# dfki-asr/morphablegraphs

Measured on AMD Instinct MI355X. Metric: motion-primitive samples scored+back-projected/sec; fraction of HBM roofline, higher is better.
Workload: dtype f32; 1 GPU; walk primitive L=40 F=156 D=79 NB=31 GMM k=8, batch=8192 candidates/GPU (BASELINE.json configs[1]); candidates_per_gpu=8192, global_candidates=8192, collective=none, clock_ramp_steps=1500

## Files before the change

morphablegraphs_amd/csrc/mg_frames_direct.hip:

```cpp
#include "mg_frames_common.h"

struct mg_direct_args {
    const float *Et32;
    const double *Et64;
    const double *mean;
    const void *lat;
    const int32_t *i0;
    const double *w;
    const float *rootm;
    void *out;
    int64_t B, ld;
    int32_t T, D, L, R, nroot;
    int32_t split;
};

template <bool LAT_F64, bool OUT_F64>
__global__ __launch_bounds__(256) void mg_frames_direct_kernel(mg_direct_args a) {
    const int64_t TD = (int64_t)a.T * a.D;
    const int64_t total = a.B * TD;
    for (int64_t idx = (int64_t)blockIdx.x * blockDim.x + threadIdx.x; idx < total; idx += (int64_t)gridDim.x * blockDim.x) {
        const int64_t b = idx / TD;
        const int o = (int)(idx - b * TD);
        const int f = o / a.D, d = o - f * a.D;
        const int i0v = a.i0[f];
        const double *wq = a.w + 4 * (size_t)f;
        const int r0 = i0v * a.D + d;
        if (!OUT_F64 && d < a.nroot && a.split) {
            float c[4];
#pragma unroll
            for (int j = 0; j < 4; j++) {
                const float *e = a.Et32 + (r0 + j * a.D);
                float acc = 0.0f;
                for (int k = 0; k < a.L; k++) acc = fmaf(e[(size_t)k * a.R], (float)mg_load_lat<LAT_F64>(a.lat, b * a.ld + k), acc);
                c[j] = acc;
            }
            float v = (float)wq[0] * c[0];
            v = fmaf((float)wq[1], c[1], v);
            v = fmaf((float)wq[2], c[2], v);
            v = fmaf((float)wq[3], c[3], v);
            const float *m = a.rootm + 8 * (size_t)f;
            ((float *)a.out)[idx] = m[d] + (m[3 + d] + v);
        } else if (OUT_F64 || d < a.nroot) {
            double c[4];
#pragma unroll
            for (int j = 0; j < 4; j++) {
                const double *e = a.Et64 + (r0 + j * a.D);
                double acc = a.mean[r0 + j * a.D];
                for (int k = 0; k < a.L; k++) acc = fma(e[(size_t)k * a.R], mg_load_lat<LAT_F64>(a.lat, b * a.ld + k), acc);
                c[j] = acc;
            }
            double v = wq[0] * c[0];
            v = fma(wq[1], c[1], v);
            v = fma(wq[2], c[2], v);
            v = fma(wq[3], c[3], v);
            if (OUT_F64) ((double *)a.out)[idx] = v;
            else ((float *)a.out)[idx] = (float)v;
        } else {
            float c[4];
#pragma unroll
            for (int j = 0; j < 4; j++) {
                const float *e = a.Et32 + (r0 + j * a.D);
                float acc = (float)a.mean[r0 + j * a.D];
                for (int k = 0; k < a.L; k++) acc = fmaf(e[(size_t)k * a.R], (float)mg_load_lat<LAT_F64>(a.lat, b * a.ld + k), acc);
                c[j] = acc;
            }
            float v = (float)wq[0] * c[0];
            v = fmaf((float)wq[1], c[1], v);
            v = fmaf((float)wq[2], c[2], v);
            v = fmaf((float)wq[3], c[3], v);
            ((float *)a.out)[idx] = v;
        }
    }
}

__global__ __launch_bounds__(256) void mg_spline_eval_kernel(const double *coeffs, const int32_t *i0, const double *w,
                                                             double *out, int64_t n, int32_t T, int32_t D, int32_t R) {
    const int64_t TD = (int64_t)T * D, total = n * TD;
    for (int64_t idx = (int64_t)blockIdx.x * blockDim.x + threadIdx.x; idx < total; idx += (int64_t)gridDim.x * blockDim.x) {
        const int64_t s = idx / TD;
        const int o = (int)(idx - s * TD);
        const int f = o / D, d = o - f * D;
        const double *c = coeffs + s * R + (size_t)i0[f] * D + d;
        const double *wq = w + 4 * (size_t)f;
        double v = wq[0] * c[0];
        v = fma(wq[1], c[D], v);
        v = fma(wq[2], c[2 * D], v);
        v = fma(wq[3], c[3 * D], v);
        out[idx] = v;
    }
}


int mg_launch_frames_direct(mg_primitive *p, const mg_time_grid *g, const void *lat, int ldt, int64_t B, int64_t ld, void *out, bool out_f64) {
    mg_direct_args a;
    a.Et32 = p->d_Et32; a.Et64 = p->d_Et64; a.mean = p->d_mean; a.lat = lat; a.i0 = g->d_i0; a.w = g->d_w; a.out = out;
    a.rootm = g->d_rootm; a.split = (!out_f64 && mg_frames_root_split(p)) ? 1 : 0;
    a.B = B; a.ld = ld; a.T = g->T; a.D = p->D; a.L = p->L; a.R = p->R; a.nroot = p->nroot;
    int64_t total = B * (int64_t)g->T * p->D;
    int64_t blocks = (total + 255) / 256;
    int grid = (int)std::min<int64_t>(blocks, (int64_t)p->ctx->n_cu * 32);
    hipStream_t st = p->ctx->stream;
    const bool lf = (ldt == MG_F64);
    if (lf && out_f64) hipLaunchKernelGGL((mg_frames_direct_kernel<true, true>), dim3(grid), dim3(256), 0, st, a);
    else if (lf) hipLaunchKernelGGL((mg_frames_direct_kernel<true, false>), dim3(grid), dim3(256), 0, st, a);
    else if (out_f64) hipLaunchKernelGGL((mg_frames_direct_kernel<false, true>), dim3(grid), dim3(256), 0, st, a);
    else hipLaunchKernelGGL((mg_frames_direct_kernel<false, false>), dim3(grid), dim3(256), 0, st, a);
    MG_HIP_CHECK(hipGetLastError());
    return MG_OK;
}

int mg_launch_spline_eval(mg_primitive *p, const mg_time_grid *g, const double *coeffs, int64_t n, double *out) {
    int64_t total = n * (int64_t)g->T * p->D;
    int grid = (int)std::min<int64_t>((total + 255) / 256, (int64_t)p->ctx->n_cu * 32);
    hipLaunchKernelGGL(mg_spline_eval_kernel, dim3(grid), dim3(256), 0, p->ctx->stream, coeffs, g->d_i0, g->d_w, out, n, g->T, p->D, p->R);
    MG_HIP_CHECK(hipGetLastError());
    return MG_OK;
}
```

Before: 108.5 million samples/s.

## Add LDS-staged batched f64 frame kernel that reuses coefficients across candidates

Adds a new f64-output path in which each block handles up to four candidates. The block stages their latents and the spline weights in LDS, computes the full coefficient vector (mean plus Et·z) once per candidate into LDS, then evaluates the 4-tap spline from LDS with paired 16-byte stores. Before, every output element recomputed four L-length dot products from global memory. This removes that redundant FMA and load traffic, at the cost of large LDS use (up to 80KB), lower occupancy and a one-time attribute setup. It only runs when the output is f64 and the batch is at least 64.

```diff
diff --git a/morphablegraphs_amd/csrc/mg_frames_direct.hip b/morphablegraphs_amd/csrc/mg_frames_direct.hip
--- a/morphablegraphs_amd/csrc/mg_frames_direct.hip
+++ b/morphablegraphs_amd/csrc/mg_frames_direct.hip
@@ -71,6 +71,166 @@
             ((float *)a.out)[idx] = v;
         }
     }
+}
+
+#define MG_F64B_BLOCK 512
+#define MG_F64B_MAX_C 4
+#define MG_F64B_RJ 2
+#define MG_F64B_KU 8
+#define MG_F64B_MIN_BATCH 64
+#define MG_F64B_LDS_BUDGET (80 * 1024)
+
+typedef double f64x2 __attribute__((ext_vector_type(2)));
+
+static size_t mg_f64b_lds_bytes(int C, int T, int L, int R) {
+    const int CP = (C + 1) & ~1;
+    return (size_t)T * 32 + (size_t)L * CP * 8 + (size_t)C * R * 8 + (size_t)T * 4;
+}
+
+__device__ __forceinline__ double mg_f64b_tap(const double *cb, const double *ws, const int *off, int f, int d, int D) {
+    const f64x2 w01 = *(const f64x2 *)(ws + 4 * f), w23 = *(const f64x2 *)(ws + 4 * f + 2);
+    const double *c = cb + off[f] + d;
+    double v = w01[0] * c[0];
+    v = fma(w01[1], c[D], v);
+    v = fma(w23[0], c[2 * D], v);
+    v = fma(w23[1], c[3 * D], v);
+    return v;
+}
+
+template <int C, bool LAT_F64>
+__global__ __launch_bounds__(MG_F64B_BLOCK) void mg_frames_f64_batch_kernel(const double *__restrict__ Et64,
+                                                                            const double *__restrict__ mean,
+                                                                            const void *__restrict__ lat, const int32_t *__restrict__ i0,
+                                                                            const double *__restrict__ w, double *__restrict__ out,
+                                                                            int64_t B, int64_t ld, int T, int D, int L, int R) {
+    constexpr int CP = (C + 1) & ~1;
+    extern __shared__ __attribute__((aligned(16))) unsigned char smem[];
+    double *ws = (double *)smem;
+    double *s = ws + 4 * (size_t)T;
+    double *cp = s + (size_t)L * CP;
+    int *off = (int *)(cp + (size_t)C * R);
+    const int tid = threadIdx.x;
+    const int64_t b0 = (int64_t)blockIdx.x * C;
+    const int nc = (int)((B - b0) < C ? (B - b0) : C);
+    for (int i = tid; i < L * CP; i += MG_F64B_BLOCK) {
+        const int k = i / CP, c = i - k * CP;
+        s[i] = c < nc ? mg_load_lat<LAT_F64>(lat, (b0 + c) * ld + k) : 0.0;
+    }
+    for (int f = tid; f < T; f += MG_F64B_BLOCK) {
+        off[f] = i0[f] * D;
+#pragma unroll
+        for (int q = 0; q < 4; q++) ws[4 * f + q] = w[4 * (size_t)f + q];
+    }
+    __syncthreads();
+    for (int rb = 0; rb < R; rb += MG_F64B_BLOCK * MG_F64B_RJ) {
+        int r[MG_F64B_RJ];
+        double acc[MG_F64B_RJ][C];
+#pragma unroll
+        for (int j = 0; j < MG_F64B_RJ; j++) {
+            const int rj = rb + j * MG_F64B_BLOCK + tid;
+            r[j] = rj < R ? rj : R - 1;
+            const double m = mean[r[j]];
+#pragma unroll
+            for (int c = 0; c < C; c++) acc[j][c] = m;
+        }
+        auto steps = [&](const double *e, int k, auto ku) {
+            constexpr int KU = decltype(ku)::value;
+            double ev[KU][MG_F64B_RJ];
+#pragma unroll
+            for (int u = 0; u < KU; u++)
+#pragma unroll
+                for (int j = 0; j < MG_F64B_RJ; j++) ev[u][j] = e[(size_t)u * R + r[j]];
+#pragma unroll
+            for (int u = 0; u < KU; u++) {
+                f64x2 sv[CP / 2];
+#pragma unroll
+                for (int q = 0; q < CP / 2; q++) sv[q] = *(const f64x2 *)(s + (k + u) * CP + 2 * q);
+#pragma unroll
+                for (int j = 0; j < MG_F64B_RJ; j++)
+#pragma unroll
+                    for (int c = 0; c < C; c++) acc[j][c] = fma(ev[u][j], sv[c >> 1][c & 1], acc[j][c]);
+            }
+        };
+        const double *e = Et64;
+        int k = 0;
+        for (; k + MG_F64B_KU <= L; k += MG_F64B_KU, e += (size_t)MG_F64B_KU * R) steps(e, k, std::integral_constant<int, MG_F64B_KU>());
+        for (; k < L; k++, e += R) steps(e, k, std::integral_constant<int, 1>());
+#pragma unroll
+        for (int j = 0; j < MG_F64B_RJ; j++) {
+            if (rb + j * MG_F64B_BLOCK + tid < R) {
+#pragma unroll
+                for (int c = 0; c < C; c++) cp[(size_t)c * R + r[j]] = acc[j][c];
+            }
+        }
+    }
+    __syncthreads();
+    const int TD = T * D;
+    const int sf = (2 * MG_F64B_BLOCK) / D, sd = 2 * MG_F64B_BLOCK - sf * D;
+    for (int c = 0; c < nc; c++) {
+        double *ob = out + (b0 + c) * (int64_t)TD;
+        const double *cb = cp + (size_t)c * R;
+        const int head = (int)(((uintptr_t)ob >> 3) & 1);
+        const int npairs = (TD - head) >> 1;
+        if (tid == MG_F64B_BLOCK - 1 && head) ob[0] = mg_f64b_tap(cb, ws, off, 0, 0, D);
+        if (tid == MG_F64B_BLOCK - 2 && ((TD - head) & 1)) ob[TD - 1] = mg_f64b_tap(cb, ws, off, T - 1, D - 1, D);
+        int e = head + 2 * tid;
+        int f = e / D, d = e - f * D;
+        for (int p = tid; p < npairs; p += MG_F64B_BLOCK) {
+            int f1 = f, d1 = d + 1;
+            if (d1 == D) { d1 = 0; f1++; }
+            f64x2 v;
+            v[0] = mg_f64b_tap(cb, ws, off, f, d, D);
+            v[1] = mg_f64b_tap(cb, ws, off, f1, d1, D);
+            *(f64x2 *)(ob + e) = v;
+            e += 2 * MG_F64B_BLOCK;
+            f += sf; d += sd;
+            if (d >= D) { d -= D; f++; }
+        }
+    }
+}
+
+static int mg_f64b_candidates(const mg_primitive *p, const mg_time_grid *g, int64_t B) {
+    if (B < MG_F64B_MIN_BATCH || (int64_t)g->T * p->D > (int64_t)INT32_MAX / 2) return 0;
+    int cmax = 0;
+    for (int c = 1; c <= MG_F64B_MAX_C; c++)
+        if (mg_f64b_lds_bytes(c, g->T, p->L, p->R) <= MG_F64B_LDS_BUDGET) cmax = c;
+    if (cmax == 0) return 0;
+    const int64_t per_cu = B / std::max(1, p->ctx->n_cu);
+    return (int)std::min<int64_t>(cmax, std::max<int64_t>(1, per_cu));
+}
+
+template <int C>
+static void mg_f64b_launch(mg_primitive *p, const mg_time_grid *g, const void *lat, bool lat_f64, int64_t B, int64_t ld, double *out) {
+    const size_t lds = mg_f64b_lds_bytes(C, g->T, p->L, p->R);
+    const unsigned grid = (unsigned)((B + C - 1) / C);
+#define MG_F64B_ARGS (const double *)p->d_Et64, (const double *)p->d_mean, lat, (const int32_t *)g->d_i0, (const double *)g->d_w, out, B, ld, (int)g->T, (int)p->D, (int)p->L, (int)p->R
+    if (lat_f64) hipLaunchKernelGGL((mg_frames_f64_batch_kernel<C, true>), dim3(grid), dim3(MG_F64B_BLOCK), lds, p->ctx->stream, MG_F64B_ARGS);
+    else hipLaunchKernelGGL((mg_frames_f64_batch_kernel<C, false>), dim3(grid), dim3(MG_F64B_BLOCK), lds, p->ctx->stream, MG_F64B_ARGS);
+#undef MG_F64B_ARGS
+}
+
+template <int C>
+static hipError_t mg_f64b_attributes() {
+    hipError_t e = hipFuncSetAttribute((const void *)mg_frames_f64_batch_kernel<C, true>, hipFuncAttributeMaxDynamicSharedMemorySize, MG_F64B_LDS_BUDGET);
+    if (e != hipSuccess) return e;
+    return hipFuncSetAttribute((const void *)mg_frames_f64_batch_kernel<C, false>, hipFuncAttributeMaxDynamicSharedMemorySize, MG_F64B_LDS_BUDGET);
+}
+
+static int mg_launch_frames_f64_batch(mg_primitive *p, const mg_time_grid *g, const void *lat, int ldt, int64_t B, int64_t ld, double *out, int C) {
+    if (!(p->ctx->attr_traj & 16u)) {
+        MG_HIP_CHECK(mg_f64b_attributes<1>());
+        MG_HIP_CHECK(mg_f64b_attributes<2>());
+        MG_HIP_CHECK(mg_f64b_attributes<3>());
+        MG_HIP_CHECK(mg_f64b_attributes<4>());
+        p->ctx->attr_traj |= 16u;
+    }
+    const bool lf = (ldt == MG_F64);
+    if (C == 1) mg_f64b_launch<1>(p, g, lat, lf, B, ld, out);
+    else if (C == 2) mg_f64b_launch<2>(p, g, lat, lf, B, ld, out);
+    else if (C == 3) mg_f64b_launch<3>(p, g, lat, lf, B, ld, out);
+    else mg_f64b_launch<4>(p, g, lat, lf, B, ld, out);
+    MG_HIP_CHECK(hipGetLastError());
+    return MG_OK;
 }
 
 __global__ __launch_bounds__(256) void mg_spline_eval_kernel(const double *coeffs, const int32_t *i0, const double *w,
@@ -92,6 +252,10 @@
 
 
 int mg_launch_frames_direct(mg_primitive *p, const mg_time_grid *g, const void *lat, int ldt, int64_t B, int64_t ld, void *out, bool out_f64) {
+    if (out_f64) {
+        const int C = mg_f64b_candidates(p, g, B);
+        if (C > 0) return mg_launch_frames_f64_batch(p, g, lat, ldt, B, ld, (double *)out, C);
+    }
     mg_direct_args a;
     a.Et32 = p->d_Et32; a.Et64 = p->d_Et64; a.mean = p->d_mean; a.lat = lat; a.i0 = g->d_i0; a.w = g->d_w; a.out = out;
     a.rootm = g->d_rootm; a.split = (!out_f64 && mg_frames_root_split(p)) ? 1 : 0;
```

After: 104.4 million samples/s. 0.962x the previous value.
